# tpy001/VFMSeg

Measured on AMD Instinct MI355X. Metric: train images/sec @512x512 DINOv2-L+LoRA (dg_lora_dinov2_ms_masked, 1024^2 sample = LR+HR 512^2 passes), higher is better.
Workload: dtype bf16; 1 GPU; configs[1]: dg_lora_dinov2_ms_masked.py, synthetic 1024^2 19-class samples -> 2x512^2 passes, bs=2/GPU, full train step (fwd+bwd+allreduce+AdamW), LoRA dropout on; global_batch=2, parallelism=dp1

## Files before the change

vfmseg_amd/csrc/gemm_bf16.hip:

```cpp
#include "gemm_launch.h"

template <int BM, int BN, int WM_W, int WN_W, int NS>
struct Cfg {
  static constexpr int WAVES = WM_W * WN_W;
  static constexpr int THREADS = WAVES * 64;
  static constexpr int A_BYTES = BM * BK * 2, B_BYTES = BN * BK * 2;
  static constexpr int STAGE_BYTES = A_BYTES + B_BYTES;
  static constexpr int A_PIECES = BM / 8 / WAVES, B_PIECES = BN / 8 / WAVES;
  static constexpr int PIECES = A_PIECES + B_PIECES;
  static constexpr int WM = BM / WM_W, WN = BN / WN_W;
  static constexpr int MI = WM / 32, NI = WN / 32;
  static constexpr int EPI_LD = WN + 4;
  static constexpr int EPI_BYTES = WAVES * 32 * EPI_LD * 4;
  static constexpr int SMEM = (NS * STAGE_BYTES > EPI_BYTES) ? NS * STAGE_BYTES : EPI_BYTES;
  static_assert(BM % (8 * WAVES) == 0 && BN % (8 * WAVES) == 0, "tile rows must split into whole DMA pieces per wave");
  static_assert(WM % 32 == 0 && WN % 32 == 0, "wave tile must be a multiple of the 32x32 MFMA");
};

typedef short s16x4 __attribute__((ext_vector_type(4)));

__device__ __attribute__((aligned(16))) unsigned char g_zero_row[512];
template <int BM, int BN, int WM_W, int WN_W, int NS, bool VEC, bool BT, bool AT = false>
__global__ void __launch_bounds__(WM_W* WN_W * 64)
    k_gemm_bf16(const bf16_t* __restrict__ A, long lda, const bf16_t* __restrict__ B, long ldb, long M, long N, long K,
                long stride_a, long stride_b, long stride_c, int tiles_m, int tiles_n, long kb_rows, EpiParams e, SkinnyTail sk) {
  using C = Cfg<BM, BN, WM_W, WN_W, NS>;
  extern __shared__ __attribute__((aligned(16))) char smem[];
  if constexpr (!BT && C::THREADS == 512 && C::SMEM >= 65536) {
    if (sk.nblk > 0 && (int)blockIdx.x >= tiles_m * tiles_n) {
      skinny_tile(sk.A, sk.lda, B, ldb, sk.M, N, K, (long)((int)blockIdx.x - tiles_m * tiles_n) * 32, sk.e, 0, smem);
      return;
    }
  }
  const int tid = threadIdx.x, lane = tid & 63;
  const int wave = __builtin_amdgcn_readfirstlane(tid >> 6);
  const int wm = wave / WN_W, wn = wave % WN_W;

  const int ntiles = tiles_m * tiles_n;
  int bid = blockIdx.x;
  {
    const int q = ntiles >> 3, r = ntiles & 7, xcd = bid & 7, idx = bid >> 3;
    bid = (xcd < r ? xcd * (q + 1) : r * (q + 1) + (xcd - r) * q) + idx;
  }
  constexpr int GM = 8;
  const int group = bid / (GM * tiles_n);
  const int first_m = group * GM;
  const int gsz = min(tiles_m - first_m, GM);
  const int tm = first_m + (bid % (GM * tiles_n)) % gsz;
  const int tn = (bid % (GM * tiles_n)) / gsz;
  const long m0 = (long)tm * BM, n0 = (long)tn * BN;
  const long z = blockIdx.y;
  const bf16_t* Ab = A + z * stride_a;
  const bf16_t* Bb = B + z * stride_b;
  long kb_valid = K;
  if constexpr (BT) {
    if (kb_rows > 0) {
      kb_valid = kb_rows - (ldb > 0 ? z * (stride_b / ldb) : 0);
      if (kb_valid > K) kb_valid = K;
      if (kb_valid < 1) kb_valid = 1;
    } else if (kb_rows < 0) {
      kb_valid = -kb_rows;
      if (kb_valid > K) kb_valid = K;
    }
  }

  const int lr = lane >> 3, pc = lane & 7;
  const bf16_t* a_src[C::A_PIECES];
  const bf16_t* b_src[C::B_PIECES];
  int at_row[C::A_PIECES];
#pragma unroll
  for (int j = 0; j < C::A_PIECES; ++j) {
    if constexpr (!AT) {
      const int r = (wave * C::A_PIECES + j) * 8 + lr;
      long gm = m0 + r;
      if (gm > M - 1) gm = M - 1;
      a_src[j] = Ab + gm * lda + ((pc ^ ((r >> 1) & 7)) << 3);
    } else {
      static_assert(!AT || (BT && BM == 128), "transposed-A path: BM = 128 (256-byte LDS rows), together with transposed B");
      const int piece = wave * C::A_PIECES + j;
      const int r = piece * 4 + (lane >> 4);
      const int c = (lane & 15) ^ ((r & 3) << 2);
      long gm = m0 + c * 8;
      if (gm > M - 8) gm = M - 8;
      at_row[j] = r;
      a_src[j] = Ab + gm;
    }
  }
  int bt_row[C::B_PIECES];
#pragma unroll
  for (int j = 0; j < C::B_PIECES; ++j) {
    if constexpr (!BT) {
      const int r = (wave * C::B_PIECES + j) * 8 + lr;
      long gn = n0 + r;
      if (gn > N - 1) gn = N - 1;
      b_src[j] = Bb + gn * ldb + ((pc ^ ((r >> 1) & 7)) << 3);
    } else {
      static_assert(!BT || BN == 128, "transposed-B path is built for BN = 128 (256-byte LDS rows)");
      const int piece = wave * C::B_PIECES + j;
      const int r = piece * 4 + (lane >> 4);
      const int c = (lane & 15) ^ ((r & 3) << 2);
      long gn = n0 + c * 8;
      if (gn > N - 8) gn = N - 8;
      bt_row[j] = r;
      b_src[j] = Bb + gn;
    }
  }
  auto stage = [&](int slot, long k0) {
    char* sa = smem + slot * C::STAGE_BYTES;
    char* sb = sa + C::A_BYTES;
#pragma unroll
    for (int j = 0; j < C::A_PIECES; ++j) {
      if constexpr (!AT) {
        glds16(a_src[j] + k0, sa + (wave * C::A_PIECES + j) * 1024);
      } else {
        const long kr = k0 + at_row[j];
        const bf16_t* src = kr < kb_valid ? a_src[j] + kr * lda : reinterpret_cast<const bf16_t*>(g_zero_row) + (lane & 15) * 8;
        glds16(src, sa + (wave * C::A_PIECES + j) * 1024);
      }
    }
#pragma unroll
    for (int j = 0; j < C::B_PIECES; ++j) {
      if constexpr (!BT) {
        glds16(b_src[j] + k0, sb + (wave * C::B_PIECES + j) * 1024);
      } else {
        long kr = k0 + bt_row[j];
        if (kr > kb_valid - 1) kr = kb_valid - 1;
        glds16(b_src[j] + kr * ldb, sb + (wave * C::B_PIECES + j) * 1024);
      }
    }
  };

  f32x16 acc[C::MI][C::NI];
#pragma unroll
  for (int i = 0; i < C::MI; ++i)
#pragma unroll
    for (int j = 0; j < C::NI; ++j)
#pragma unroll
      for (int r = 0; r < 16; ++r) acc[i][j][r] = 0.f;

  const int fr = lane & 31, fh = lane >> 5;
  int a_off[C::MI], a_sw[C::MI], b_off[C::NI], b_sw[C::NI];
#pragma unroll
  for (int i = 0; i < C::MI; ++i) {
    const int r = wm * C::WM + i * 32 + fr;
    a_off[i] = r * 128;
    a_sw[i] = (r >> 1) & 7;
  }
#pragma unroll
  for (int j = 0; j < C::NI; ++j) {
    const int r = wn * C::WN + j * 32 + fr;
    b_off[j] = r * 128;
    b_sw[j] = (r >> 1) & 7;
  }

  const int nk = (int)(K / BK);
#pragma unroll
  for (int s = 0; s < NS - 1; ++s)
    if (s < nk) stage(s, (long)s * BK);

  for (int t = 0; t < nk; ++t) {
    const int inflight = min(NS - 2, nk - 1 - t);
    if (inflight >= NS - 2 && NS >= 2) wait_vmcnt<(NS - 2) * C::PIECES>();
    else if (NS >= 4 && inflight == NS - 3) wait_vmcnt<(NS >= 3 ? (NS - 3) : 0) * C::PIECES>();
    else if (NS >= 5 && inflight == NS - 4) wait_vmcnt<(NS >= 4 ? (NS - 4) : 0) * C::PIECES>();
    else wait_vmcnt<0>();
    __builtin_amdgcn_s_barrier();
    if (t + NS - 1 < nk) stage((t + NS - 1) % NS, (long)(t + NS - 1) * BK);
    const char* sa = smem + (t % NS) * C::STAGE_BYTES;
    const char* sb = sa + C::A_BYTES;
    auto read_b = [&](int s2, int j) -> bf16x8 {
      if constexpr (!BT) {
        return *reinterpret_cast<const bf16x8*>(sb + b_off[j] + (((2 * s2 + fh) ^ b_sw[j]) << 4));
      } else {
        const int g = lane >> 4, i2 = lane & 15, q = i2 >> 2, p = i2 & 3, h2 = g >> 1;
        const int chunk = (wn * C::WN + j * 32) / 8 + 2 * (g & 1) + (p >> 1);
        const int r0 = 16 * s2 + 8 * h2 + q, r1 = r0 + 4;
        const s16x4 lo = __builtin_amdgcn_ds_read_tr16_b64_v4i16(
            (__attribute__((address_space(3))) s16x4*)(sb + r0 * 256 + ((chunk ^ ((r0 & 3) << 2)) << 4) + ((p & 1) << 3)));
        const s16x4 hi = __builtin_amdgcn_ds_read_tr16_b64_v4i16(
            (__attribute__((address_space(3))) s16x4*)(sb + r1 * 256 + ((chunk ^ ((r1 & 3) << 2)) << 4) + ((p & 1) << 3)));
        union { struct { s16x4 a, b; } st; bf16x8 v; } u;
        u.st.a = lo;
        u.st.b = hi;
        return u.v;
      }
    };
    auto read_a = [&](int s2, int i) -> bf16x8 {
      if constexpr (!AT) {
        return *reinterpret_cast<const bf16x8*>(sa + a_off[i] + (((2 * s2 + fh) ^ a_sw[i]) << 4));
      } else {
        const int g = lane >> 4, i2 = lane & 15, q = i2 >> 2, p = i2 & 3, h2 = g >> 1;
        const int chunk = (wm * C::WM + i * 32) / 8 + 2 * (g & 1) + (p >> 1);
        const int r0 = 16 * s2 + 8 * h2 + q, r1 = r0 + 4;
        const s16x4 lo = __builtin_amdgcn_ds_read_tr16_b64_v4i16(
            (__attribute__((address_space(3))) s16x4*)(sa + r0 * 256 + ((chunk ^ ((r0 & 3) << 2)) << 4) + ((p & 1) << 3)));
        const s16x4 hi = __builtin_amdgcn_ds_read_tr16_b64_v4i16(
            (__attribute__((address_space(3))) s16x4*)(sa + r1 * 256 + ((chunk ^ ((r1 & 3) << 2)) << 4) + ((p & 1) << 3)));
        union { struct { s16x4 a, b; } st; bf16x8 v; } u;
        u.st.a = lo;
        u.st.b = hi;
        return u.v;
      }
    };
    bf16x8 af[2][C::MI], bfr[2][C::NI];
#pragma unroll
    for (int i = 0; i < C::MI; ++i) af[0][i] = read_a(0, i);
#pragma unroll
    for (int j = 0; j < C::NI; ++j) bfr[0][j] = read_b(0, j);
#pragma unroll
    for (int s = 0; s < BK / 16; ++s) {
      const int cur = s & 1, nxt = cur ^ 1;
      if (s + 1 < BK / 16) {
#pragma unroll
        for (int i = 0; i < C::MI; ++i)
          af[nxt][i] = read_a(s + 1, i);
#pragma unroll
        for (int j = 0; j < C::NI; ++j) bfr[nxt][j] = read_b(s + 1, j);
      }
#pragma unroll
      for (int i = 0; i < C::MI; ++i)
#pragma unroll
        for (int j = 0; j < C::NI; ++j)
          acc[i][j] = VFM_MFMA16(af[cur][i], bfr[cur][j], acc[i][j]);
    }
  }

  const long zoff = z * stride_c;
  __syncthreads();
  float* img = reinterpret_cast<float*>(smem) + wave * 32 * C::EPI_LD;
  if constexpr (VEC) epi_wave_tile<C::MI, C::NI, 1>(e, zoff, acc, img, lane, m0 + wm * C::WM, n0 + wn * C::WN, M, N);
  else epi_scalar<C::MI, C::NI, 1>(e, zoff, acc, img, lane, m0 + wm * C::WM, n0 + wn * C::WN, M, N);
}

template <int BM, int BN, int WM_W, int WN_W, int NS, bool VEC, bool BT, bool AT = false>
static void launch_one(const vfm_gemm_desc* d, hipStream_t s, const vfm_gemm_desc* tail = nullptr) {
  using C = Cfg<BM, BN, WM_W, WN_W, NS>;
  const int tiles_m = cdiv(d->M, BM), tiles_n = cdiv(d->N, BN);
  const long batch = d->batch > 0 ? d->batch : 1;
  static bool attr = false;
  if (!attr) {
    (void)hipFuncSetAttribute((const void*)k_gemm_bf16<BM, BN, WM_W, WN_W, NS, VEC, BT, AT>, hipFuncAttributeMaxDynamicSharedMemorySize, C::SMEM);
    attr = true;
  }
  const SkinnyTail sk = skinny_tail(tail);
  dim3 grid(tiles_m * tiles_n + sk.nblk, (unsigned)batch), blk(C::THREADS);
  const long ldb = BT ? d->sb_k : d->sb_n;
  const long kb_rows = d->kb_rows;
  hipLaunchKernelGGL((k_gemm_bf16<BM, BN, WM_W, WN_W, NS, VEC, BT, AT>), grid, blk, C::SMEM, s, (const bf16_t*)d->A, AT ? d->sa_k : d->sa_m,
                     (const bf16_t*)d->B, ldb, d->M, d->N, d->K, d->stride_a, d->stride_b, d->stride_c, tiles_m, tiles_n, kb_rows,
                     make_epi(d), sk);
}

template <int ID, int BM, int BN, int WM_W, int WN_W, int NS>
static void launch_two_stage(const vfm_gemm_desc* d, hipStream_t s, const GemmPlan& p, const vfm_gemm_desc* tail) {
  using C = Cfg<BM, BN, WM_W, WN_W, NS>;
  static_assert(kGemmConfigs[gemm_config_index(ID)].hosts_tail == (C::THREADS == 512 && C::SMEM >= 65536), "config table: hosts_tail");
  if (p.vec) launch_one<BM, BN, WM_W, WN_W, NS, true, false>(d, s, tail);
  else launch_one<BM, BN, WM_W, WN_W, NS, false, false>(d, s, tail);
}
void vfm_gemm_launch_10(const vfm_gemm_desc* d, hipStream_t s, const GemmPlan& p, const vfm_gemm_desc* tail) { launch_two_stage<10, 64, 64, 2, 2, 4>(d, s, p, tail); }
void vfm_gemm_launch_16(const vfm_gemm_desc* d, hipStream_t s, const GemmPlan& p, const vfm_gemm_desc* tail) { launch_two_stage<16, 256, 256, 4, 4, 2>(d, s, p, tail); }
void vfm_gemm_launch_17(const vfm_gemm_desc* d, hipStream_t s, const GemmPlan& p, const vfm_gemm_desc* tail) { launch_two_stage<17, 128, 128, 2, 4, 2>(d, s, p, tail); }
void vfm_gemm_launch_18(const vfm_gemm_desc* d, hipStream_t s, const GemmPlan& p, const vfm_gemm_desc* tail) { launch_two_stage<18, 64, 128, 2, 2, 2>(d, s, p, tail); }

template <int BM, int WM_W, int WN_W, int NS = 2>
static void launch_bt(const vfm_gemm_desc* d, hipStream_t s, bool vec) {
  if (vec) launch_one<BM, 128, WM_W, WN_W, NS, true, true>(d, s);
  else launch_one<BM, 128, WM_W, WN_W, NS, false, true>(d, s);
}

__global__ void __launch_bounds__(512) k_gemm_bf16_skinny(const bf16_t* __restrict__ A, long lda, const bf16_t* __restrict__ B, long ldb,
                                                          long M, long N, long K, long stride_a, long stride_b, long stride_c,
                                                          EpiParams e) {
  __shared__ __attribute__((aligned(16))) char stg[65536];
  const long z = blockIdx.y;
  skinny_tile(A + z * stride_a, lda, B + z * stride_b, ldb, M, N, K, (long)blockIdx.x * 32, e, z * stride_c, stg);
}

static void launch_skinny(const vfm_gemm_desc* d, hipStream_t s) {
  const long batch = d->batch > 0 ? d->batch : 1;
  hipLaunchKernelGGL(k_gemm_bf16_skinny, dim3(cdiv(d->N, 32), (unsigned)batch), dim3(512), 0, s, (const bf16_t*)d->A, d->sa_m,
                     (const bf16_t*)d->B, d->sb_n, d->M, d->N, d->K, d->stride_a, d->stride_b, d->stride_c, make_epi(d));
}

GemmKnobs g_gemm_knobs;
long g_nt_bytes = 0;

typedef void (*GemmLaunch)(const vfm_gemm_desc*, hipStream_t, const GemmPlan&, const vfm_gemm_desc*);
#define VFM_GEMM_LAUNCHER(id, family, min_k, span, hosts, deep, msg) vfm_gemm_launch_##id,
static const GemmLaunch kGemmLaunch[] = {VFM_GEMM_CONFIGS(VFM_GEMM_LAUNCHER)};
#undef VFM_GEMM_LAUNCHER

int vfm_gemm_bf16_impl(const vfm_gemm_desc* d0, hipStream_t s) {
  const GemmPlan p = gemm_select(*d0, g_gemm_knobs);
  if (p.err) VFM_FAIL(p.err, "vfm_gemm(bf16): %s (gemm_cfg %d)", kGemmMsgs[p.msg], g_gemm_knobs.force_cfg);
  vfm_gemm_desc dm, dt;
  const vfm_gemm_desc* d = d0;
  if (p.tail_rows > 0) {
    dm = *d0, dt = *d0;
    const long mm = d0->M - p.tail_rows;
    dm.M = mm;
    dt.M = p.tail_rows;
    auto adv = [&](const void* ptr, int dt_, long ld) -> const void* {
      return ptr ? (const void*)((const char*)ptr + mm * ld * (dt_ == VFM_BF16 || dt_ == VFM_SPLIT3 ? 2 : 4)) : nullptr;
    };
    dt.A = adv(d0->A, VFM_BF16, d0->sa_m);
    dt.C = (void*)adv(d0->C, d0->c_dt, d0->ldc);
    dt.residual = adv(d0->residual, d0->r_dt, d0->ldr);
    dt.aux = adv(d0->aux, d0->aux_dt, d0->ld_aux);
    dt.C2 = (void*)adv(d0->C2, d0->c2_dt, d0->ldc2);
    d = &dm;
  }
  const vfm_gemm_desc* ride = (p.tail_mode == GEMM_TAIL_BLOCKS || p.tail_mode == GEMM_TAIL_INSIDE) ? &dt : nullptr;
  switch (p.kind) {
    case GEMM_SKINNY: launch_skinny(d, s); break;
    case GEMM_BT64: launch_bt<64, 1, 4>(d, s, p.vec); break;
    case GEMM_BT128: launch_bt<128, 2, 4>(d, s, p.vec); break;
    case GEMM_ATBT:
      if (p.vec) launch_one<128, 128, 2, 4, 2, true, true, true>(d, s);
      else launch_one<128, 128, 2, 4, 2, false, true, true>(d, s);
      break;
    default: kGemmLaunch[gemm_config_index(p.cfg)](d, s, p, ride); break;
  }
  if (p.tail_mode == GEMM_TAIL_SEPARATE) launch_skinny(&dt, s);
  return VFM_OK;
}
```

vfmseg_amd/csrc/gemm_select.h:

```cpp
#pragma once
#include <stdint.h>
#include "../../include/vfmseg_hip.h"

struct GemmKnobs {
  int force_cfg = -1;
  int split_tail = 3;
  int batch_tiles = 1;
  int bt64 = 1;
  int fold_tail = 1;
  int use_pp = 184;
  int use_ps = 0;
  int use_192 = 3;
  int w44_k = 1024;
  int deep_sep_k = 0;
  int deep_tail_k = 0;
};
extern GemmKnobs g_gemm_knobs;
extern long g_nt_bytes;
extern int g_pp_dbg;
extern int g_ps_burst;

#ifdef VFM_EXPERIMENTAL_GEMM
constexpr bool kGemmExperimental = true;
#else
constexpr bool kGemmExperimental = false;
#endif

enum GemmFamily { GEMM_FAM_TWO_STAGE, GEMM_FAM_PP, GEMM_FAM_RING, GEMM_FAM_SPLITK, GEMM_FAM_PS, GEMM_FAM_V5 };
enum GemmMsg {
  GEMM_MSG_NONE, GEMM_MSG_UNKNOWN, GEMM_MSG_RETIRED, GEMM_MSG_EXPERIMENT, GEMM_MSG_PP256, GEMM_MSG_PP128, GEMM_MSG_RING256, GEMM_MSG_DEEP,
  GEMM_MSG_SPLITK, GEMM_MSG_W44, GEMM_MSG_T192, GEMM_MSG_V5, GEMM_MSG_PS2, GEMM_MSG_PS1
};
constexpr const char* kGemmMsgs[] = {
    "",
    "unknown config",
    "retired config: the two-stage sweep configs 0-9, 11-15 and 19-29 are no longer built (live: 10, 16, 17, 18)",
    "gemm_ps.hip / gemm_v5.hip (configs 37, 38, 50) are experiments: build with VFMSEG_EXPERIMENTAL=1",
    "the ping-pong kernel needs K >= 128",
    "the 128x128 ping-pong kernel needs K >= 256",
    "the 64-wide-K-tile ring kernels need K >= 128 and operands spanning < 4 GiB",
    "the deep-ring 128x128 kernels need K >= 256 and operands spanning < 4 GiB",
    "the split-K ring kernel needs K % 128 == 0, K >= 512, one batch, <= 512 tiles of 128 x 128, a 16-byte aligned epilogue",
    "the 4-wave 128x128 kernel needs K >= 128 and operands spanning < 4 GiB",
    "the 192x256 kernel needs K >= 128 and operands spanning < 4 GiB",
    "the 16x16x32 256x256 kernel needs K >= 128 and operands spanning < 4 GiB",
    "the persistent kernel needs M % 256 == 0, N % 256 == 0, K % 64 == 0, K >= 576 and a bf16 bias / GELU / multiply epilogue",
    "the persistent kernel needs M % 256 == 0, N % 128 == 0, K % 64 == 0, K >= 576 and a bf16 bias / GELU / multiply epilogue",
};

#define VFM_GEMM_CONFIGS_SHIPPED(X)                                  \
  X(10, GEMM_FAM_TWO_STAGE, 0, 0, false, false, GEMM_MSG_NONE)       \
  X(16, GEMM_FAM_TWO_STAGE, 0, 0, false, false, GEMM_MSG_NONE)       \
  X(17, GEMM_FAM_TWO_STAGE, 0, 0, true, false, GEMM_MSG_NONE)        \
  X(18, GEMM_FAM_TWO_STAGE, 0, 0, false, false, GEMM_MSG_NONE)       \
  X(30, GEMM_FAM_PP, 128, 0, true, false, GEMM_MSG_PP256)            \
  X(31, GEMM_FAM_PP, 256, 0, true, false, GEMM_MSG_PP128)            \
  X(32, GEMM_FAM_RING, 128, 256, true, false, GEMM_MSG_RING256)      \
  X(33, GEMM_FAM_RING, 128, 256, true, false, GEMM_MSG_RING256)      \
  X(34, GEMM_FAM_RING, 128, 256, true, false, GEMM_MSG_RING256)      \
  X(35, GEMM_FAM_RING, 256, 256, true, true, GEMM_MSG_DEEP)          \
  X(36, GEMM_FAM_RING, 256, 256, true, true, GEMM_MSG_DEEP)          \
  X(39, GEMM_FAM_RING, 128, 256, true, false, GEMM_MSG_T192)         \
  X(40, GEMM_FAM_RING, 128, 256, true, false, GEMM_MSG_T192)         \
  X(51, GEMM_FAM_SPLITK, 512, 256, true, false, GEMM_MSG_SPLITK)     \
  X(52, GEMM_FAM_RING, 128, 256, true, false, GEMM_MSG_W44)
#ifdef VFM_EXPERIMENTAL_GEMM
#define VFM_GEMM_CONFIGS(X)                                          \
  VFM_GEMM_CONFIGS_SHIPPED(X)                                        \
  X(37, GEMM_FAM_PS, 576, 256, true, false, GEMM_MSG_PS2)            \
  X(38, GEMM_FAM_PS, 576, 256, true, false, GEMM_MSG_PS1)            \
  X(50, GEMM_FAM_V5, 128, 256, true, false, GEMM_MSG_V5)
#else
#define VFM_GEMM_CONFIGS(X) VFM_GEMM_CONFIGS_SHIPPED(X)
#endif

struct GemmConfig {
  int id, family, min_k, span;
  bool hosts_tail, deep_ring;
  int msg;
};
#define VFM_GEMM_ROW(id, family, min_k, span, hosts, deep, msg) {id, family, min_k, span, hosts, deep, msg},
constexpr GemmConfig kGemmConfigs[] = {VFM_GEMM_CONFIGS(VFM_GEMM_ROW)};
#undef VFM_GEMM_ROW
constexpr int kGemmConfigCount = (int)(sizeof(kGemmConfigs) / sizeof(kGemmConfigs[0]));
constexpr int gemm_config_index(int id) {
  for (int i = 0; i < kGemmConfigCount; ++i)
    if (kGemmConfigs[i].id == id) return i;
  return -1;
}
constexpr bool gemm_config_retired(int id) { return id >= 0 && id <= 29 && gemm_config_index(id) < 0; }
constexpr bool gemm_config_experimental(int id) { return id == 37 || id == 38 || id == 50; }

enum GemmKind { GEMM_SKINNY = 0, GEMM_BT64 = 1, GEMM_BT128 = 2, GEMM_ATBT = 3, GEMM_TILE = 4 };
enum GemmTail {
  GEMM_TAIL_NONE = 0,
  GEMM_TAIL_BLOCKS = 1,
  GEMM_TAIL_INSIDE = 2,
  GEMM_TAIL_SEPARATE = 3,
  GEMM_TAIL_ROW_TILE = 4
};
struct GemmPlan {
  int err = VFM_OK;
  int msg = GEMM_MSG_NONE;
  int kind = GEMM_SKINNY;
  int cfg = -1;
  int vec = 0;
  long tail_rows = 0;
  int tail_mode = GEMM_TAIL_NONE;
};

inline int gemm_cdiv(long a, long b) { return (int)((a + b - 1) / b); }

inline bool gemm_vec_ok(const vfm_gemm_desc& d) {
  auto a16 = [](const void* p) { return ((uintptr_t)p % 16) == 0; };
  const long bm = d.bias_mod > 0 ? d.bias_mod : d.N;
  bool ok = (d.N % 4 == 0) && (d.ldc % 4 == 0) && a16(d.C) && (d.stride_c % 4 == 0);
  if (d.bias) ok = ok && a16(d.bias) && (bm % 4 == 0);
  if (d.colscale) ok = ok && a16(d.colscale);
  if (d.residual) ok = ok && a16(d.residual) && (d.ldr % 4 == 0);
  if (d.aux) ok = ok && a16(d.aux) && (d.ld_aux % 4 == 0);
  if (d.C2) ok = ok && a16(d.C2) && (d.ldc2 % 4 == 0);
  return ok;
}

constexpr int GEMM_SPLITK_TILES = 512;
inline bool gemm_splitk_ok(const vfm_gemm_desc& d, bool vec) {
  return vec && d.batch <= 1 && d.K % 128 == 0 && d.K >= 512 && (long)gemm_cdiv(d.M, 128) * gemm_cdiv(d.N, 128) <= GEMM_SPLITK_TILES;
}

enum { PS_BIAS = 0, PS_GELU_DGELU = 1, PS_MUL = 2, PS_GELU = 3 };
constexpr int PS_PEEL = 8;
inline int gemm_ps_kind(const vfm_gemm_desc* d) {
  auto a16 = [](const void* p) { return ((uintptr_t)p % 16) == 0; };
  if (d->c_dt != VFM_BF16 || d->residual || d->colscale || !a16(d->C) || d->ldc % 8) return -1;
  const long bm = d->bias_mod > 0 ? d->bias_mod : d->N;
  if (d->bias && (!a16(d->bias) || bm % 4 || bm < d->N)) return -1;
  switch (d->ep_mode) {
    case VFM_EP_NONE: return (d->bias && !d->C2) ? PS_BIAS : -1;
    case VFM_EP_GELU: return (d->bias && !d->C2) ? PS_GELU : -1;
    case VFM_EP_GELU_DGELU: return (d->bias && d->C2 && d->c2_dt == VFM_BF16 && a16(d->C2) && d->ldc2 % 8 == 0) ? PS_GELU_DGELU : -1;
    case VFM_EP_MUL: return (!d->bias && !d->C2 && d->aux && d->aux_dt == VFM_BF16 && a16(d->aux) && d->ld_aux % 8 == 0) ? PS_MUL : -1;
    default: return -1;
  }
}
inline bool gemm_ps_ok(const vfm_gemm_desc* d, int per) {
  if (!kGemmExperimental || gemm_ps_kind(d) < 0 || d->batch > 1 || per < 1 || per > 2) return false;
  if (d->sa_k != 1 || d->sb_k != 1 || d->M % 256 || d->N % (128 * per) || d->K % 64 || d->K < 64 * (PS_PEEL + 1)) return false;
  if ((d->M + 256) * d->sa_m >= (1l << 31) || (d->N + 256) * d->sb_n >= (1l << 31)) return false;
  if ((d->M + 8) * d->ldc >= (1l << 31) * 2 || (d->aux && (d->M + 8) * d->ld_aux >= (1l << 31))) return false;
  return ((uintptr_t)d->A % 16) == 0 && ((uintptr_t)d->B % 16) == 0 && d->sa_m % 8 == 0 && d->sb_n % 8 == 0;
}

inline bool gemm_span_ok(const vfm_gemm_desc& d, long span) {
  return (d.M + span) * d.sa_m < (1l << 31) && (d.N + span) * d.sb_n < (1l << 31);
}

inline GemmPlan gemm_plan_error(int err, int msg) {
  GemmPlan p;
  p.err = err, p.msg = msg;
  return p;
}

inline GemmPlan gemm_select_main(const vfm_gemm_desc& d, const GemmKnobs& kn, long tail_rows, bool has_tail) {
  GemmPlan p;
  p.vec = gemm_vec_ok(d);
  p.tail_rows = tail_rows;
  if (d.sb_n == 1 && d.sb_k != 1) {
    if (d.sa_m == 1 && d.sa_k != 1) {
      p.kind = GEMM_ATBT;
      return p;
    }
    const bool few = (long)gemm_cdiv(d.M, 128) * gemm_cdiv(d.N, 128) * (d.batch > 0 ? d.batch : 1) < 128;
    p.kind = (d.M <= 64 || (kn.bt64 && few)) ? GEMM_BT64 : GEMM_BT128;
    return p;
  }
  const bool tail = has_tail;
  bool separate = tail_rows > 0 && !has_tail;
  int cfg = kn.force_cfg;
  if (cfg < 0) {
    const long nbatch = d.batch > 0 ? d.batch : 1;
    const long t128 = (long)gemm_cdiv(d.M, 128) * gemm_cdiv(d.N, 128) * (kn.batch_tiles ? nbatch : 1);
    const long t256 = (long)gemm_cdiv(d.M, 256) * gemm_cdiv(d.N, 256);
    const bool span31 = gemm_span_ok(d, 128);
    const bool span33 = gemm_span_ok(d, 256);
    const long t192 = (long)gemm_cdiv(d.M, 192) * gemm_cdiv(d.N, 256);
    const double eff192 = (double)t192 / (256.0 * gemm_cdiv(t192, 256)), eff256 = (double)t256 / (256.0 * gemm_cdiv(t256, 256));
    const bool big_m = d.M >= 8192 && d.N >= 1024 && d.K >= 1024 && nbatch == 1 && span33 && !(kn.use_pp & 64);
    const long t64 = (long)gemm_cdiv(d.M, 64) * gemm_cdiv(d.N, 64);
    if (d.N <= 32) cfg = 10;
    else if ((kn.use_192 & 1) && big_m && eff192 >= eff256 + 0.08)
      cfg = 40;
    else if ((kn.use_192 & 2) && big_m && d.N >= 2048 && t256 > 256 && eff256 >= 0.8 && eff256 < 0.9)
      cfg = 33;
    else if ((kn.use_ps & 1) && d.N >= 2048 && t256 >= 224 && t256 % 256 == 0 && d.K >= 1024 && gemm_ps_ok(&d, 2))
      cfg = 37;
    else if (!(kn.use_pp & 64) && tail && t128 >= 96 && t128 <= 160 && d.N >= 512 && d.K >= 1024 && span31 && nbatch == 1)
      cfg = 31;
    else if (!(kn.use_pp & 64) && d.N >= 1024 && d.N < 2048 && t256 >= 128 && t256 <= 200 && span33 && nbatch == 1 &&
             (d.K >= 2048 || (t256 >= 170 && d.K >= 1024)))
      cfg = 33;
    else if (!(kn.use_pp & 64) && d.N >= 4096 && t256 >= 700 && t256 < 768 && d.K >= 1024 && span33 && nbatch == 1)
      cfg = 33;
    else if (!(kn.use_pp & 64) && d.N >= 2048 && t256 >= 224 && t256 <= 256 && d.K >= 1024 && span33 && nbatch == 1 && !tail)
      cfg = 33;
    else if (t128 <= 160 && d.K >= 512 && t64 <= 544)
      cfg = 10;
    else if (t128 <= 160) cfg = 18;
    else if ((kn.use_pp & 2) && t128 > 160 && t128 <= 272 && d.K >= 256 && span31)
      cfg = 31;
    else if ((kn.use_pp & 128) && d.N >= 2048 && t256 >= 176 && t256 < 256 && d.K >= 512 && span33 && nbatch == 1)
      cfg = 33;
    else if ((kn.use_pp & 16) && d.N >= 2048 && (t256 % 256 == 0 || t256 >= 768) && d.K >= 128 && span33)
      cfg = 33;
    else if (d.N >= 2048 && (t256 % 256 == 0 || t256 >= 768) && !(kn.use_pp & 8))
      cfg = ((kn.use_pp & 1) && d.K >= 128 && span33) ? 30 : 16;
    else cfg = 17;
    if (cfg == 17 && (kn.use_pp & 32) && d.K >= 128 && span31)
      cfg = 34;
    if (cfg == 34 && kn.w44_k > 0 && d.K >= kn.w44_k) cfg = 52;
    if (cfg == 34 && !tail && t128 <= 256 && d.K >= 256 && d.M % 128 == 0) cfg = 35;
    if (cfg == 34 && tail && t128 <= 256 && d.M % 128 == 0 && d.K >= kn.deep_tail_k && kn.deep_tail_k > 0) cfg = 35;
    if (cfg == 34 && tail && t128 <= 256 && d.M % 128 == 0 && d.K >= 256 && kn.deep_sep_k > 0 && d.K >= kn.deep_sep_k) cfg = 35, separate = true;
  }
  const int row = gemm_config_index(cfg);
  if (row < 0) {
    if (gemm_config_experimental(cfg)) return gemm_plan_error(VFM_E_UNSUPPORTED, GEMM_MSG_EXPERIMENT);
    if (gemm_config_retired(cfg)) return gemm_plan_error(VFM_E_UNSUPPORTED, GEMM_MSG_RETIRED);
    return gemm_plan_error(VFM_E_INVAL, GEMM_MSG_UNKNOWN);
  }
  const GemmConfig& c = kGemmConfigs[row];
  bool ok = d.K >= c.min_k && (c.span == 0 || (d.K % 64 == 0 && gemm_span_ok(d, c.span)));
  if (c.family == GEMM_FAM_SPLITK) ok = ok && gemm_splitk_ok(d, p.vec);
  if (c.family == GEMM_FAM_PS) ok = gemm_ps_ok(&d, cfg == 37 ? 2 : 1);
  if (!ok) return gemm_plan_error(VFM_E_UNSUPPORTED, c.msg);
  p.kind = GEMM_TILE, p.cfg = cfg;
  if (c.family == GEMM_FAM_SPLITK || c.family == GEMM_FAM_PS) p.vec = 1;
  if (tail_rows > 0) {
    if (separate || !c.hosts_tail) p.tail_mode = GEMM_TAIL_SEPARATE;
    else if (c.deep_ring && tail_rows <= 8 && d.sa_k == 1) p.tail_mode = GEMM_TAIL_INSIDE;
    else p.tail_mode = GEMM_TAIL_BLOCKS;
  }
  return p;
}

inline GemmPlan gemm_select(const vfm_gemm_desc& d0, const GemmKnobs& kn) {
  const long tail = d0.M % 128;
  const bool bt = (d0.sb_n == 1 && d0.sb_k != 1);
  if (bt) return gemm_select_main(d0, kn, 0, false);
  const long t128m = (long)((d0.M - tail) / 128) * gemm_cdiv(d0.N, 128);
  const bool pp_coarse = !(kn.use_pp & 64) && tail > 0 && t128m >= 96 && t128m <= 160 && d0.N >= 512 && d0.K >= 1024 && d0.batch <= 1;
  const bool rows64 = !pp_coarse && d0.N > 32 && d0.K >= 512 && (long)gemm_cdiv(d0.M, 128) * gemm_cdiv(d0.N, 128) <= 160 &&
                      (long)gemm_cdiv(d0.M, 64) * gemm_cdiv(d0.N, 64) <= 544;
  const bool peelable = kn.split_tail && d0.M > 512 && tail > 0 && tail <= 32 && (d0.batch <= 1);
  if (peelable && !(rows64 && (kn.split_tail & 2))) {
    vfm_gemm_desc dm = d0;
    dm.M = d0.M - tail;
    return gemm_select_main(dm, kn, tail, kn.fold_tail != 0);
  }
  if (d0.M <= 32 && d0.N >= 32) return GemmPlan();
  GemmPlan p = gemm_select_main(d0, kn, 0, false);
  if (peelable && !p.err) p.tail_mode = GEMM_TAIL_ROW_TILE;
  return p;
}
```

vfmseg_amd/csrc/tune.hip:

```cpp
#include <limits.h>
#include "attn_common.h"
#include "gemm_select.h"

#ifndef VFM_EXPERIMENTAL_GEMM
int g_ps_burst = 0;
#endif

namespace {
int g_nt_mb = 0;
struct Knob { const char* key; int* value; int lo, hi; };
const Knob kKnobs[] = {
    {"gemm_cfg", &g_gemm_knobs.force_cfg, INT_MIN, INT_MAX},
    {"gemm_use_pp", &g_gemm_knobs.use_pp, INT_MIN, INT_MAX},
    {"gemm_use_ps", &g_gemm_knobs.use_ps, INT_MIN, INT_MAX},
    {"gemm_use_192", &g_gemm_knobs.use_192, INT_MIN, INT_MAX},
    {"gemm_w44_k", &g_gemm_knobs.w44_k, 0, INT_MAX},
    {"gemm_deep_sep_k", &g_gemm_knobs.deep_sep_k, 0, INT_MAX},
    {"gemm_deep_tail_k", &g_gemm_knobs.deep_tail_k, INT_MIN, INT_MAX},
    {"gemm_batch_tiles", &g_gemm_knobs.batch_tiles, INT_MIN, INT_MAX},
    {"gemm_bt64", &g_gemm_knobs.bt64, INT_MIN, INT_MAX},
    {"gemm_fold_tail", &g_gemm_knobs.fold_tail, INT_MIN, INT_MAX},
    {"gemm_split_tail", &g_gemm_knobs.split_tail, INT_MIN, INT_MAX},
    {"gemm_nt_mb", &g_nt_mb, INT_MIN, INT_MAX},
    {"pp_dbg", &g_pp_dbg, INT_MIN, INT_MAX},
    {"ps_burst", &g_ps_burst, INT_MIN, INT_MAX},
    {"attn_short_grid", &g_attn_short_grid, INT_MIN, INT_MAX},
    {"attn_il", &g_attn_il, 0, 3},
    {"attn_xcd", &g_attn_xcd, INT_MIN, INT_MAX},
    {"attn_fwd64", &g_attn_fwd64, INT_MIN, INT_MAX},
    {"attn_lds_pad", &g_attn_lds_pad, INT_MIN, INT_MAX},
};
}

extern "C" int vfm_tune(const char* key, int value) {
  for (const Knob& k : kKnobs) {
    if (!key || strcmp(key, k.key) != 0) continue;
    if (value < k.lo || value > k.hi) VFM_FAIL(VFM_E_INVAL, "vfm_tune(%s): %d is outside %d .. %d", k.key, value, k.lo, k.hi);
    *k.value = value;
    g_nt_bytes = (long)g_nt_mb << 20;
    return VFM_OK;
  }
  VFM_FAIL(VFM_E_INVAL, "vfm_tune: unknown key");
}
```

Measured before the change: 135.7 images/s.

## Pick GEMM LDS ring depth at launch from grid size and use raw DMA for BT paths

Configs 17/18 and the transposed-B and AT/BT GEMM paths now choose a 2-, 3- or 4-stage LDS ring at launch. A 4-deep ring is used when the grid fits within one wave of CUs, to hide more global-load latency in under-filled grids. Transposed-B kernels also issue global_load_lds through a hand-written inline asm that sets m0 directly, to cut per-load overhead. The cost is more instantiated kernels, more LDS per block (lower occupancy when depth is 4), and a tuning knob gemm_ring.

```diff
diff --git a/vfmseg_amd/csrc/gemm_bf16.hip b/vfmseg_amd/csrc/gemm_bf16.hip
--- a/vfmseg_amd/csrc/gemm_bf16.hip
+++ b/vfmseg_amd/csrc/gemm_bf16.hip
@@ -20,7 +20,13 @@
 typedef short s16x4 __attribute__((ext_vector_type(4)));
 
 __device__ __attribute__((aligned(16))) unsigned char g_zero_row[512];
-template <int BM, int BN, int WM_W, int WN_W, int NS, bool VEC, bool BT, bool AT = false>
+
+__device__ __forceinline__ void glds16_raw(const void* g, void* l) {
+  const unsigned la = (unsigned)(uintptr_t)(__attribute__((address_space(3))) void*)l;
+  asm volatile("s_mov_b32 m0, %1\n\ts_nop 0\n\tglobal_load_lds_dwordx4 %0, off" ::"v"(g), "s"(la) : "memory", "m0");
+}
+
+template <int BM, int BN, int WM_W, int WN_W, int NS, bool VEC, bool BT, bool AT = false, bool RAW = BT>
 __global__ void __launch_bounds__(WM_W* WN_W * 64)
     k_gemm_bf16(const bf16_t* __restrict__ A, long lda, const bf16_t* __restrict__ B, long ldb, long M, long N, long K,
                 long stride_a, long stride_b, long stride_c, int tiles_m, int tiles_n, long kb_rows, EpiParams e, SkinnyTail sk) {
@@ -105,27 +111,31 @@
       b_src[j] = Bb + gn;
     }
   }
+  auto dma = [&](const void* src, char* dst) {
+    if constexpr (RAW) glds16_raw(src, dst);
+    else glds16(src, dst);
+  };
   auto stage = [&](int slot, long k0) {
     char* sa = smem + slot * C::STAGE_BYTES;
     char* sb = sa + C::A_BYTES;
 #pragma unroll
     for (int j = 0; j < C::A_PIECES; ++j) {
       if constexpr (!AT) {
-        glds16(a_src[j] + k0, sa + (wave * C::A_PIECES + j) * 1024);
+        dma(a_src[j] + k0, sa + (wave * C::A_PIECES + j) * 1024);
       } else {
         const long kr = k0 + at_row[j];
         const bf16_t* src = kr < kb_valid ? a_src[j] + kr * lda : reinterpret_cast<const bf16_t*>(g_zero_row) + (lane & 15) * 8;
-        glds16(src, sa + (wave * C::A_PIECES + j) * 1024);
+        dma(src, sa + (wave * C::A_PIECES + j) * 1024);
       }
     }
 #pragma unroll
     for (int j = 0; j < C::B_PIECES; ++j) {
       if constexpr (!BT) {
-        glds16(b_src[j] + k0, sb + (wave * C::B_PIECES + j) * 1024);
+        dma(b_src[j] + k0, sb + (wave * C::B_PIECES + j) * 1024);
       } else {
         long kr = k0 + bt_row[j];
         if (kr > kb_valid - 1) kr = kb_valid - 1;
-        glds16(b_src[j] + kr * ldb, sb + (wave * C::B_PIECES + j) * 1024);
+        dma(b_src[j] + kr * ldb, sb + (wave * C::B_PIECES + j) * 1024);
       }
     }
   };
@@ -232,41 +242,92 @@
   else epi_scalar<C::MI, C::NI, 1>(e, zoff, acc, img, lane, m0 + wm * C::WM, n0 + wn * C::WN, M, N);
 }
 
-template <int BM, int BN, int WM_W, int WN_W, int NS, bool VEC, bool BT, bool AT = false>
+template <int BM, int BN, int WM_W, int WN_W, int NS, bool VEC, bool BT, bool AT = false, bool RAW = BT>
 static void launch_one(const vfm_gemm_desc* d, hipStream_t s, const vfm_gemm_desc* tail = nullptr) {
   using C = Cfg<BM, BN, WM_W, WN_W, NS>;
   const int tiles_m = cdiv(d->M, BM), tiles_n = cdiv(d->N, BN);
   const long batch = d->batch > 0 ? d->batch : 1;
   static bool attr = false;
   if (!attr) {
-    (void)hipFuncSetAttribute((const void*)k_gemm_bf16<BM, BN, WM_W, WN_W, NS, VEC, BT, AT>, hipFuncAttributeMaxDynamicSharedMemorySize, C::SMEM);
+    (void)hipFuncSetAttribute((const void*)k_gemm_bf16<BM, BN, WM_W, WN_W, NS, VEC, BT, AT, RAW>, hipFuncAttributeMaxDynamicSharedMemorySize, C::SMEM);
     attr = true;
   }
   const SkinnyTail sk = skinny_tail(tail);
   dim3 grid(tiles_m * tiles_n + sk.nblk, (unsigned)batch), blk(C::THREADS);
   const long ldb = BT ? d->sb_k : d->sb_n;
   const long kb_rows = d->kb_rows;
-  hipLaunchKernelGGL((k_gemm_bf16<BM, BN, WM_W, WN_W, NS, VEC, BT, AT>), grid, blk, C::SMEM, s, (const bf16_t*)d->A, AT ? d->sa_k : d->sa_m,
+  hipLaunchKernelGGL((k_gemm_bf16<BM, BN, WM_W, WN_W, NS, VEC, BT, AT, RAW>), grid, blk, C::SMEM, s, (const bf16_t*)d->A, AT ? d->sa_k : d->sa_m,
                      (const bf16_t*)d->B, ldb, d->M, d->N, d->K, d->stride_a, d->stride_b, d->stride_c, tiles_m, tiles_n, kb_rows,
                      make_epi(d), sk);
+}
+
+int g_gemm_ring = 0;
+
+static int gemm_cu_count() {
+  static int cus[64];
+  int dev = 0;
+  if (hipGetDevice(&dev) != hipSuccess || dev < 0 || dev >= 64) return 256;
+  if (!cus[dev]) {
+    int n = 0;
+    if (hipDeviceGetAttribute(&n, hipDeviceAttributeMultiprocessorCount, dev) != hipSuccess || n <= 0) n = 256;
+    cus[dev] = n;
+  }
+  return cus[dev];
+}
+
+static int gemm_ring_depth(long blocks, long nk) {
+  if (g_gemm_ring >= 2 && g_gemm_ring <= 4) return g_gemm_ring;
+  if (g_gemm_ring == 1) return 2;
+  int ns = blocks <= gemm_cu_count() ? 4 : 2;
+  if (ns > nk + 1) ns = nk + 1 < 2 ? 2 : (int)(nk + 1);
+  return ns;
+}
+
+template <int BM, int BN, int WM_W, int WN_W, bool BT, bool AT>
+static void launch_ring(const vfm_gemm_desc* d, hipStream_t s, bool vec, const vfm_gemm_desc* tail = nullptr) {
+  const long blocks = ((long)cdiv(d->M, BM) * cdiv(d->N, BN) + (tail ? cdiv(tail->N, 32) : 0)) * (d->batch > 0 ? d->batch : 1);
+  if constexpr (BT) {
+    if (g_gemm_ring == 1) {
+      if (vec) launch_one<BM, BN, WM_W, WN_W, 2, true, BT, AT, false>(d, s, tail);
+      else launch_one<BM, BN, WM_W, WN_W, 2, false, BT, AT, false>(d, s, tail);
+      return;
+    }
+  }
+  switch (gemm_ring_depth(blocks, d->K / BK)) {
+    case 4:
+      if (vec) launch_one<BM, BN, WM_W, WN_W, 4, true, BT, AT>(d, s, tail);
+      else launch_one<BM, BN, WM_W, WN_W, 4, false, BT, AT>(d, s, tail);
+      break;
+    case 3:
+      if (vec) launch_one<BM, BN, WM_W, WN_W, 3, true, BT, AT>(d, s, tail);
+      else launch_one<BM, BN, WM_W, WN_W, 3, false, BT, AT>(d, s, tail);
+      break;
+    default:
+      if (vec) launch_one<BM, BN, WM_W, WN_W, 2, true, BT, AT>(d, s, tail);
+      else launch_one<BM, BN, WM_W, WN_W, 2, false, BT, AT>(d, s, tail);
+      break;
+  }
 }
 
 template <int ID, int BM, int BN, int WM_W, int WN_W, int NS>
 static void launch_two_stage(const vfm_gemm_desc* d, hipStream_t s, const GemmPlan& p, const vfm_gemm_desc* tail) {
   using C = Cfg<BM, BN, WM_W, WN_W, NS>;
   static_assert(kGemmConfigs[gemm_config_index(ID)].hosts_tail == (C::THREADS == 512 && C::SMEM >= 65536), "config table: hosts_tail");
-  if (p.vec) launch_one<BM, BN, WM_W, WN_W, NS, true, false>(d, s, tail);
-  else launch_one<BM, BN, WM_W, WN_W, NS, false, false>(d, s, tail);
+  if constexpr (ID == 17 || ID == 18) {
+    launch_ring<BM, BN, WM_W, WN_W, false, false>(d, s, p.vec, tail);
+  } else {
+    if (p.vec) launch_one<BM, BN, WM_W, WN_W, NS, true, false>(d, s, tail);
+    else launch_one<BM, BN, WM_W, WN_W, NS, false, false>(d, s, tail);
+  }
 }
 void vfm_gemm_launch_10(const vfm_gemm_desc* d, hipStream_t s, const GemmPlan& p, const vfm_gemm_desc* tail) { launch_two_stage<10, 64, 64, 2, 2, 4>(d, s, p, tail); }
 void vfm_gemm_launch_16(const vfm_gemm_desc* d, hipStream_t s, const GemmPlan& p, const vfm_gemm_desc* tail) { launch_two_stage<16, 256, 256, 4, 4, 2>(d, s, p, tail); }
 void vfm_gemm_launch_17(const vfm_gemm_desc* d, hipStream_t s, const GemmPlan& p, const vfm_gemm_desc* tail) { launch_two_stage<17, 128, 128, 2, 4, 2>(d, s, p, tail); }
 void vfm_gemm_launch_18(const vfm_gemm_desc* d, hipStream_t s, const GemmPlan& p, const vfm_gemm_desc* tail) { launch_two_stage<18, 64, 128, 2, 2, 2>(d, s, p, tail); }
 
-template <int BM, int WM_W, int WN_W, int NS = 2>
+template <int BM, int WM_W, int WN_W>
 static void launch_bt(const vfm_gemm_desc* d, hipStream_t s, bool vec) {
-  if (vec) launch_one<BM, 128, WM_W, WN_W, NS, true, true>(d, s);
-  else launch_one<BM, 128, WM_W, WN_W, NS, false, true>(d, s);
+  launch_ring<BM, 128, WM_W, WN_W, true, false>(d, s, vec);
 }
 
 __global__ void __launch_bounds__(512) k_gemm_bf16_skinny(const bf16_t* __restrict__ A, long lda, const bf16_t* __restrict__ B, long ldb,
@@ -316,10 +377,7 @@
     case GEMM_SKINNY: launch_skinny(d, s); break;
     case GEMM_BT64: launch_bt<64, 1, 4>(d, s, p.vec); break;
     case GEMM_BT128: launch_bt<128, 2, 4>(d, s, p.vec); break;
-    case GEMM_ATBT:
-      if (p.vec) launch_one<128, 128, 2, 4, 2, true, true, true>(d, s);
-      else launch_one<128, 128, 2, 4, 2, false, true, true>(d, s);
-      break;
+    case GEMM_ATBT: launch_ring<128, 128, 2, 4, true, true>(d, s, p.vec); break;
     default: kGemmLaunch[gemm_config_index(p.cfg)](d, s, p, ride); break;
   }
   if (p.tail_mode == GEMM_TAIL_SEPARATE) launch_skinny(&dt, s);
diff --git a/vfmseg_amd/csrc/gemm_select.h b/vfmseg_amd/csrc/gemm_select.h
--- a/vfmseg_amd/csrc/gemm_select.h
+++ b/vfmseg_amd/csrc/gemm_select.h
@@ -17,6 +17,7 @@
 };
 extern GemmKnobs g_gemm_knobs;
 extern long g_nt_bytes;
+extern int g_gemm_ring;
 extern int g_pp_dbg;
 extern int g_ps_burst;
 
diff --git a/vfmseg_amd/csrc/tune.hip b/vfmseg_amd/csrc/tune.hip
--- a/vfmseg_amd/csrc/tune.hip
+++ b/vfmseg_amd/csrc/tune.hip
@@ -22,6 +22,7 @@
     {"gemm_fold_tail", &g_gemm_knobs.fold_tail, INT_MIN, INT_MAX},
     {"gemm_split_tail", &g_gemm_knobs.split_tail, INT_MIN, INT_MAX},
     {"gemm_nt_mb", &g_nt_mb, INT_MIN, INT_MAX},
+    {"gemm_ring", &g_gemm_ring, 0, 4},
     {"pp_dbg", &g_pp_dbg, INT_MIN, INT_MAX},
     {"ps_burst", &g_ps_burst, INT_MIN, INT_MAX},
     {"attn_short_grid", &g_attn_short_grid, INT_MIN, INT_MAX},
```

Result: no change. 136.5 images/s (median of 6 runs) (+0.6%).
